# imuncle/TSCM_Calib

Hardware: AMD Instinct MI355X
Metric: LM iterations/sec at 4 cams x 10k views (joint intrinsics+extrinsics, fp64) (higher is better)
Workload: dtype f64

## Files before the change

### tscm_calib_amd/csrc/tscm_kernels.h

```cpp
#pragma once

#include "tscm_math.h"
#include "tscm_fastmath.h"
#include "tscm_nd_plan.h"
#include "tscm_layout.h"
#include "tscm_exec_plan.h"
#include "tscm_columns.h"
#include "tscm_ctrl.h"

namespace tscm {

static_assert(kColFree == kFA && kColGrad == kFR, "tscm_columns.h plans the columns of tscm_math.h's camera tile");
constexpr int kWcolTc = 3;
constexpr int kFac = 56;
constexpr int kFacM = 0;
constexpr int kFacC = 15;
constexpr int kFacL = 21;
constexpr int kFacI = 36;
constexpr int kFacZ = 42;
constexpr int kFacD = 48;
constexpr int kTcols = 15;
constexpr int kTcWb = 0, kTcWc = 4, kTcF = 8, kTcOne = 9, kTcXi = 10, kTcLam = 12, kTcAl = 13, kTcR = 14;
__host__ __device__ constexpr int tc_tc(int j) { return 3 + 4 * j; }
constexpr int kVConst = 27;
// ... 1500 lines not shown
    S.pairpart[(size_t)256 * P.pc_tile[pc] + t] = (red[0][t] + red[1][t]) + (red[2][t] + red[3][t]);
}

template <int ENTRIES>
__device__ __forceinline__ void t_reduce_block(const DevState &S, int bid, int part, int cb, int ce, double (*red)[ENTRIES])
{
    const int e = threadIdx.x % ENTRIES, slice = threadIdx.x / ENTRIES;
    const int entry = part * ENTRIES + e;
    const int per = (ce - cb + kTSlices - 1) / kTSlices;
    const int b0 = cb + slice * per, b1 = min(ce, b0 + per);
    double a0 = 0.0, a1 = 0.0, a2 = 0.0, a3 = 0.0, a4 = 0.0, a5 = 0.0, a6 = 0.0, a7 = 0.0;
    const double *src = S.pairpart + entry;
    for (int c = b0; c < b1; c += 8) {
        const double v0 = src[(size_t)256 * c];
        const double v1 = c + 1 < b1 ? src[(size_t)256 * (c + 1)] : 0.0;
        const double v2 = c + 2 < b1 ? src[(size_t)256 * (c + 2)] : 0.0;
        const double v3 = c + 3 < b1 ? src[(size_t)256 * (c + 3)] : 0.0;
        const double v4 = c + 4 < b1 ? src[(size_t)256 * (c + 4)] : 0.0;
        const double v5 = c + 5 < b1 ? src[(size_t)256 * (c + 5)] : 0.0;
        const double v6 = c + 6 < b1 ? src[(size_t)256 * (c + 6)] : 0.0;
        const double v7 = c + 7 < b1 ? src[(size_t)256 * (c + 7)] : 0.0;
        a0 += v0; a1 += v1; a2 += v2; a3 += v3; a4 += v4; a5 += v5; a6 += v6; a7 += v7;
    }
    red[slice][e] = ((a0 + a1) + (a2 + a3)) + ((a4 + a5) + (a6 + a7));
    __syncthreads();
    if (slice == 0) {
        double v[kTSlices];
#pragma unroll
        for (int q = 0; q < kTSlices; ++q) v[q] = red[q][e];
#pragma unroll
        for (int w = kTSlices / 2; w >= 1; w >>= 1)
#pragma unroll
            for (int q = 0; q < w; ++q) v[q] += v[q + w];
        handoff_store(&S.T[(size_t)256 * bid + entry], v[0]);
    }
}
__global__ __launch_bounds__(kTEntries * kTSlices) void k_T_reduce(DevProblem P, DevState S)
{
    if (S.ctrl->done) return;
    __shared__ double red[kTSlices][kTEntries];
    constexpr int kParts = 256 / kTEntries;
    const int bid = blockIdx.x / kParts;
    t_reduce_block<kTEntries>(S, bid, blockIdx.x % kParts, P.bid_part_ptr[bid], P.bid_part_ptr[bid + 1], red);
}

__device__ __forceinline__ double load_T_lut(const DevProblem &P, const double *T, int i, int j)
{
    int lo = i >> 4, hi = j >> 4, a = i & 15, b = j & 15;
    if (lo > hi) { const int t = lo; lo = hi; hi = t; const int u = a; a = b; b = u; }
    const int tile = P.bid_lut[lo * P.C + hi];
    return tile >= 0 ? T[(size_t)256 * tile + a * 16 + b] : 0.0;
}

struct TailOperands { double x, hg, hrow[kFA]; };
__device__ __forceinline__ void tail_prefetch(const DevProblem &P, const DevState &S, int cur, const double *H, TailOperands &o)
{
    const int i = threadIdx.x;
    o.x = 0.0; o.hg = 0.0;
#pragma unroll
    for (int b = 0; b < kFA; ++b) o.hrow[b] = 0.0;
    if (i < P.n_pad) {
        const int m = i >> 4, ai = i & 15;
        if (ai < 6) o.x = S.cam_rt[cur][6 * m + ai];
        else if (ai < 15) o.x = S.intr[cur][9 * m + (ai - 6)];
        if (ai < kFA) {
#pragma unroll
            for (int b = 0; b < kFA; ++b) o.hrow[b] = H[256 * m + ai * 16 + b];
            o.hg = H[256 * m + ai * 16 + kFR];
        }
    }
}
__device__ __forceinline__ void reduced_solution_tail(const DevProblem &P, const DevState &S, int cur, int fail, const TailOperands &o,
                                                      const double *yv, const double *s_sc, double *s_yh, const unsigned char *s_act, double *sred,
                                                      int publish_epoch = 0)
{
    const int n = P.n_pad, i = threadIdx.x;
    const int m = i >> 4, ai = i & 15;
    double model = 0.0, stepsq = 0.0, yh = 0.0;
    if (i < n) {
        const bool act = s_act[i] && !fail;
        yh = act ? s_sc[i] * yv[i] : 0.0;
        handoff_store(&S.yhat[i], yh);
        s_yh[i] = yh;
        if (ai < kFA) {
            const double x = o.x;
            const double xn = x + (-yh);
            if (ai < 6) handoff_store(&S.cam_rt[cur ^ 1][6 * m + ai], xn); else handoff_store(&S.intr[cur ^ 1][9 * m + (ai - 6)], xn);
            const double d = x - xn; stepsq = d * d;
        } else if (ai < 15) {
            handoff_store(&S.intr[cur ^ 1][9 * m + (ai - 6)], o.x);
        }
    }
    if (publish_epoch > 0) asm volatile("s_waitcnt vmcnt(0)" ::: "memory");
    __syncthreads();
    if (publish_epoch > 0 && i == 0) __hip_atomic_store(S.y_flag, 2 * publish_epoch + (fail ? 1 : 0), __ATOMIC_RELAXED, __HIP_MEMORY_SCOPE_AGENT);
    if (publish_epoch > 0 && i >= 64 && i < 64 + P.C) write_camera_record(S, cur ^ 1, i - 64);
    if (i < n && ai < kFA && yh != 0.0) {
        double hy = 0.0;
#pragma unroll
        for (int b = 0; b < kFA; ++b) hy += o.hrow[b] * s_yh[m * 16 + b];
        model = yh * (o.hg - 0.5 * hy);
    }
    { double red[2] = { model, stepsq }, mdummy = 0.0; block_reduce256<2>(red, mdummy, sred); model = red[0]; stepsq = red[1]; }
    if (i == 0) { S.ctrl->model_cam = model; S.ctrl->stepsq_cam = stepsq; S.ctrl->lin_fail = fail; *S.fac_fail = 0; }
}

template <int NTH, bool WAIT>
__device__ __forceinline__ void backsub_body(const DevProblem &P, const DevState &S, int with_floats, const int blk, const int nblk, const int epoch, const int t_need);

#include "tscm_solve_nd.h"
#include "tscm_solve_dense4.h"

constexpr int kBigNT = 1024;
constexpr int kBigBatch = 4;
__host__ __device__ inline size_t solve_big_lds_bytes(int N, int n_pad)
{
    return sizeof(double) * ((size_t)2 * 16 * (N + 16) + 16 * 17 + 2 * (size_t)N + 16 + 3 * (size_t)n_pad) + sizeof(int) * (size_t)N + (size_t)n_pad;
}
__device__ __forceinline__ size_t big_block(int I, int J) { return ((size_t)(I * (I + 1) / 2 + J)) << 8; }
__device__ __forceinline__ size_t big_idx(int r, int c)
{
    return big_block(r >> 4, c >> 4) + (size_t)((((c & 15) + 16 * (r & 3)) << 2) + ((r & 15) >> 2));
}
__device__ __forceinline__ double readlane_f64(double v, int lane)
{
    return __hiloint2double(__builtin_amdgcn_readlane(__double2hiint(v), lane), __builtin_amdgcn_readlane(__double2loint(v), lane));
}
__device__ __forceinline__ void lds_barrier() { asm volatile("s_waitcnt lgkmcnt(0)\n\ts_barrier" ::: "memory"); }

__global__ __launch_bounds__(kBigNT) void k_solve_reduced_big(DevProblem P, DevState S)
{
    extern __shared__ __attribute__((aligned(32))) double lds[];
    const int n = P.n_pad, na = P.n_act;
    const int N = (na + 15) & ~15, NP = N >> 4;
    const int XP = N + 16;
    double *pbuf = lds;
    double *Ld = pbuf + 2 * 16 * XP;
    double *wv = Ld + 16 * 17;
    double *idg = wv + N;
    double *yk = idg + N;
    double *yv = yk + 16;
    double *s_sc = yv + n;
    double *s_yh = s_sc + n;
    int *s_map = reinterpret_cast<int *>(s_yh + n);
    unsigned char *s_act = reinterpret_cast<unsigned char *>(s_map + N);
    __shared__ int s_fail;
    __shared__ double sred[256];
    const int tid = threadIdx.x, wave = tid >> 6, lane = tid & 63;
    if (S.ctrl->done) return;
    const int cur = S.ctrl->cur;
    const double radius = S.ctrl->radius;
    const double dmin = S.ctrl->opt.min_lm_diagonal, dmax = S.ctrl->opt.max_lm_diagonal;
    const double *H = S.H[cur];
    double *A = S.Abig;
    for (int i = tid; i < n; i += kBigNT) { s_sc[i] = S.s_c[i]; s_act[i] = P.col_active[i]; yv[i] = 0.0; }
    for (int i = tid; i < N; i += kBigNT) s_map[i] = i < na ? P.act_map[i] : -1;
    if (tid == 0) s_fail = S.ctrl->lin_fail | *S.fac_fail;
    __syncthreads();
#ifdef TSCM_BIG_PROFILE
    long long tp0 = wall_clock64(), tp_diag = 0, tp_solve = 0, tp_upd = 0;
#endif
    for (int kb = 0; wave + 16 * kb <= N; kb += 16) {
        const int rmax = min(N, wave + 16 * (kb + 15));
        for (int c = lane; c <= rmax && c < N; c += 64) {
            const int j = s_map[c];
            const int mj = j >> 4, bj = j & 15;
            const double scj = j >= 0 ? s_sc[j] : 0.0;
            double v[16];
#pragma unroll
            for (int u = 0; u < 16; ++u) {
                const int r = wave + 16 * (kb + u);
                v[u] = (r == c) ? 1.0 : 0.0;
                if (r > N || c > r) continue;
                if (r == N) {
                    v[u] = j >= 0 ? scj * (H[256 * mj + bj * 16 + kFR] - load_T_lut(P, S.T, j, mj * 16 + kFR)) : 0.0;
                } else {
                    const int i = s_map[r];
                    if (i >= 0 && j >= 0) {
                        const int mi = i >> 4, ai = i & 15;
// ... 137 lines not shown
        }
        if (wave == 0) {
#pragma unroll
            for (int u = 0; u < 4; ++u) { const int e = lane + 64 * u; Ld[(e >> 4) * 17 + (e & 15)] = ldg[u]; }
            wave_lds_fence();
            if (lane == 0) {
                double y[16];
#pragma unroll
                for (int c = 15; c >= 0; --c) {
                    double v = wv[k0 + c];
#pragma unroll
                    for (int q = c + 1; q < 16; ++q) v -= Ld[q * 17 + c] * y[q];
                    y[c] = v * idg[k0 + c];
                }
#pragma unroll
                for (int c = 0; c < 16; ++c) { yk[c] = y[c]; wv[k0 + c] = y[c]; }
            }
        }
        lds_barrier();
        if (tid < k0) {
            double v = wv[tid];
#pragma unroll
            for (int c = 0; c < 16; ++c) v -= lrow[c] * yk[c];
            wv[tid] = v;
        }
        lds_barrier();
#pragma unroll
        for (int c = 0; c < 16; ++c) lrow[c] = lnext[c];
#pragma unroll
        for (int u = 0; u < 4; ++u) ldg[u] = dnext[u];
    }
    TailOperands tail_ops;
    tail_prefetch(P, S, cur, H, tail_ops);
    for (int i = tid; i < na; i += kBigNT) yv[s_map[i]] = wv[i];
    __syncthreads();
#ifdef TSCM_BIG_PROFILE
    long long tp3 = wall_clock64();
#endif
    reduced_solution_tail(P, S, cur, s_fail, tail_ops, yv, s_sc, s_yh, s_act, sred);
#ifdef TSCM_BIG_PROFILE
    if (tid == 0) printf("big solve N=%d  build %lld  factor %lld (diag %lld solve %lld update %lld)  backsub %lld  tail %lld  [10 ns ticks]\n", N,
                         tp1 - tp0, tp2 - tp1, tp_diag, tp_solve, tp_upd, tp3 - tp2, wall_clock64() - tp3);
#endif
}

constexpr int kBsTile = 64;
template <int NTH> struct BsGeom {
    static constexpr int kBoards = NTH / 8;
    static constexpr int kPassSlots = NTH / 16;
    static constexpr int kPasses = 4;
    static constexpr int kRoundSlots = kPasses * kPassSlots;
    static constexpr int kLdsA = kRoundSlots * 6, kLdsB = kBoards * kFac, kLdsC = kBsTile * (kVFloatOff + 1);
    static constexpr int kLds = kLdsC > kLdsB ? (kLdsC > kLdsA ? kLdsC : kLdsA) : (kLdsB > kLdsA ? kLdsB : kLdsA);
    static_assert(kBoards * kFac == 7 * NTH, "the factor records are 7 doubles per thread");
    static_assert(kBoards <= 64 && 64 + kMaxCam <= NTH, "lane roles of phase B: the boards in wave 0, the cameras from wave 1 on");
};

template <int NTH, bool WAIT>
__device__ __forceinline__ void backsub_body(const DevProblem &P, const DevState &S, int with_floats, const int blk, const int nblk, const int epoch, const int t_need)
{
    constexpr int kBsBoards = BsGeom<NTH>::kBoards, kBsThreads = NTH, kPassSlots = BsGeom<NTH>::kPassSlots, kPasses = BsGeom<NTH>::kPasses, kRoundSlots = BsGeom<NTH>::kRoundSlots;
#ifndef TSCM_BS_CAM_LANE0
#define TSCM_BS_CAM_LANE0 64
#endif
    constexpr int kBsCamLane0 = TSCM_BS_CAM_LANE0;
    const int b0 = blk * kBsBoards;
    const int nbl = min(kBsBoards, P.B - b0);
    const int s0 = P.bv_ptr[b0], s1 = P.bv_ptr[b0 + nbl];
    const int ctrl_done = S.ctrl->done, cur = S.ctrl->cur;
    int fail = WAIT ? 0 : S.ctrl->lin_fail;
    if (ctrl_done) return;
    extern __shared__ __attribute__((aligned(16))) double dyn[];
    double (*s_qv)[6] = reinterpret_cast<double (*)[6]>(dyn);
    double *s_fac = dyn;
    double *st_all = dyn;
    __shared__ double s_q[kBsBoards][6], s_new[kBsBoards][6];
    __shared__ double s_yh[16 * kMaxCam];
    double (*s_rc)[12] = reinterpret_cast<double (*)[12]>(s_yh);
    static_assert(12 * kMaxCam <= 16 * kMaxCam, "s_rc aliases s_yh");
    __shared__ double sm[16];
    __shared__ int s_view[kBsTile];
    const int t = threadIdx.x;
    PHASE_STAMP(ts0);
    const int my_q0 = t < nbl ? P.bv_ptr[b0 + t] : 0, my_q1 = t < nbl ? P.bv_ptr[b0 + t + 1] : 0;
    const int c_slot = min(s0 + t, max(s1 - 1, 0));
    const int c_view = s1 > s0 ? P.slot_view[c_slot] : 0, c_board = s1 > s0 ? P.slot_board[c_slot] : 0, c_cam = s1 > s0 ? P.slot_cam[c_slot] : 0;
    double xb[6], sbv[6];
#pragma unroll
    for (int k = 0; k < 6; ++k) { xb[k] = t < nbl ? S.board_rt[cur][6 * (b0 + t) + k] : 0.0; sbv[k] = t < nbl ? S.s_b[6 * (b0 + t) + k] : 1.0; }
    double facv[7];
#pragma unroll
    for (int j = 0; j < 7; ++j) facv[j] = S.fac[(size_t)kFac * b0 + min(t + kBsThreads * j, nbl * kFac - 1)];
    if constexpr (!WAIT) { for (int i = t; i < P.n_pad; i += kBsThreads) s_yh[i] = S.yhat[i]; }
    if (t < kBsBoards * 6) (&s_q[0][0])[t] = 0.0;
    if constexpr (!WAIT) { if (t == 64) for (int m = blk; m < P.C; m += nblk) write_camera_record(S, cur ^ 1, m); }
    {
        const int grp = t >> 4, a = t & 15;
        const __amdgpu_buffer_rsrc_t r_w = make_rsrc(S.rec[cur], sizeof(double) * (size_t)kRecW * P.V);
        constexpr unsigned BAD = 0xffffe000u;
        double w[kPasses][6];
        int camv[kPasses];
        auto request = [&](int rbase) {
#pragma unroll
            for (int j = 0; j < kPasses; ++j) {
                const int slot = rbase + kPassSlots * j + grp;
                const unsigned off = (a < kFA && slot < s1) ? 8u * ((unsigned)kRecW * (unsigned)slot + 6u * (unsigned)a) : BAD;
#pragma unroll
                for (int k = 0; k < 3; ++k) { const d2 v = buf_load_2f64(r_w, off, 16u * (unsigned)k); w[j][2 * k] = v[0]; w[j][2 * k + 1] = v[1]; }
                camv[j] = P.slot_cam[min(slot, max(s1 - 1, 0))];
            }
        };
        request(s0);
        if constexpr (WAIT) {
            __shared__ int s_flag;
            if (t == 0) {
                const long long t_start = wall_clock64();
                int f;
                while (((f = __hip_atomic_load(S.y_flag, __ATOMIC_RELAXED, __HIP_MEMORY_SCOPE_AGENT)) >> 1) < epoch) {
                    __builtin_amdgcn_s_sleep(8);
                    if (wall_clock64() - t_start > kHandoffTimeoutTicks) { f = -1; break; }
                }
                if (f < 0) {
                    __hip_atomic_store(&S.ctrl->fault, 1, __ATOMIC_RELAXED, __HIP_MEMORY_SCOPE_AGENT);
                    __hip_atomic_store(&S.ctrl->term_type, 2, __ATOMIC_RELAXED, __HIP_MEMORY_SCOPE_AGENT);
                    __hip_atomic_store(&S.ctrl->done, 1, __ATOMIC_RELAXED, __HIP_MEMORY_SCOPE_AGENT);
                }
                s_flag = f;
            }
            __syncthreads();
            if (s_flag < 0 || __hip_atomic_load(&S.ctrl->done, __ATOMIC_RELAXED, __HIP_MEMORY_SCOPE_AGENT)) return;
            fail = s_flag & 1;
            for (int i = t; i < P.n_pad; i += kBsThreads) s_yh[i] = handoff_load(&S.yhat[i]);
        }
        for (int rbase = s0; rbase < s1; rbase += kRoundSlots) {
            const int rend = min(s1, rbase + kRoundSlots);
            __syncthreads();
#pragma unroll
            for (int j = 0; j < kPasses; ++j) {
                const int sl = kPassSlots * j + grp;
                const double yh = a < kFA ? s_yh[16 * camv[j] + a] : 0.0;
                double p[6];
#pragma unroll
                for (int k = 0; k < 6; ++k) {
                    p[k] = (a < kFA ? w[j][k] : 0.0) * yh;
                    p[k] = row16_allsum(p[k]);
                }
                if (a == 0) {
#pragma unroll
                    for (int k = 0; k < 6; ++k) s_qv[sl][k] = p[k];
                }
            }
            if (rbase + kRoundSlots < s1) request(rbase + kRoundSlots);
            __syncthreads();
            if (t < nbl) {
                for (int q = max(my_q0, rbase); q < min(my_q1, rend); ++q)
#pragma unroll
                    for (int k = 0; k < 6; ++k) s_q[t][k] += s_qv[q - rbase][k];
            }
        }
        __syncthreads();
#pragma unroll
        for (int j = 0; j < 7; ++j) s_fac[t + kBsThreads * j] = facv[j];
        __syncthreads();
    }
    PHASE_STAMP(ts1);
    double mb = 0.0, ss = 0.0;
    if (t < nbl) {
        const int b = b0 + t;
        if (my_q1 == my_q0 || fail) {
#pragma unroll
            for (int k = 0; k < 6; ++k) { S.board_rt[cur ^ 1][6 * b + k] = xb[k]; s_new[t][k] = xb[k]; }
        } else {
            const double *f = s_fac + kFac * t;
            double tt[6], y[6], pz[6];
#pragma unroll
            for (int i = 0; i < 6; ++i) {
                double v = f[kFacC + i] * s_q[t][i];
#pragma unroll
                for (int k = 0; k < i; ++k) v -= f[kFacM + i * (i - 1) / 2 + k] * pz[k];
                pz[i] = v;
                tt[i] = f[kFacZ + i] - v;
            }
#pragma unroll
            for (int i = 5; i >= 0; --i) {
                double w = tt[i];
#pragma unroll
                for (int k = i + 1; k < 6; ++k) w -= f[kFacL + k * (k - 1) / 2 + i] * y[k];
                y[i] = w * f[kFacI + i];
            }
#pragma unroll
            for (int k = 0; k < 6; ++k) {
                mb += 0.5 * tt[k] * tt[k] + 0.5 * f[kFacD + k] * y[k] * y[k];
                const double x = xb[k];
                const double xn = x + (-(sbv[k] * y[k]));
                const double d = x - xn;
                ss += d * d;
                S.board_rt[cur ^ 1][6 * b + k] = xn;
                s_new[t][k] = xn;
            }
        }
    } else if (t >= kBsCamLane0 && t < kBsCamLane0 + P.C) {
        const int m = t - kBsCamLane0;
        double crt[3], Rc[9], dRc[27];
        double crt6[6];
#pragma unroll
        for (int k = 0; k < 6; ++k) crt6[k] = WAIT ? handoff_load(&S.cam_rt[cur ^ 1][6 * m + k]) : S.cam_rt[cur ^ 1][6 * m + k];
        for (int k = 0; k < 3; ++k) crt[k] = crt6[k];
        rotation_and_derivatives(crt, Rc, dRc);
        for (int k = 0; k < 9; ++k) s_rc[m][k] = Rc[k];
        for (int k = 0; k < 3; ++k) s_rc[m][9 + k] = crt6[3 + k];

    }
    {
        double red[2] = { mb, ss }, mdummy = 0.0;
        block_reduce256<2>(red, mdummy, sm);
        if (t == 0) { S.bs_part[2 * blk] = red[0]; S.bs_part[2 * blk + 1] = red[1]; }
    }
    PHASE_STAMP(ts2);
    for (int base = s0; base < s1; base += kBsTile) {
        const int slot = base + t;
        int view = -1;
        if (t < kBsTile && slot < s1) {
            const bool first = base == s0;
            view = first ? c_view : P.slot_view[slot];
            const int bl = (first ? c_board : P.slot_board[slot]) - b0, m = first ? c_cam : P.slot_cam[slot];
            double rt[6], bc[kBoardConst];
#pragma unroll
            for (int k = 0; k < 6; ++k) rt[k] = s_new[bl][k];
            board_constants(rt, bc);
            double *o = st_all + (size_t)t * (kVFloatOff + 1);
            view_point_constants(s_rc[m], s_rc[m] + 9, bc, rt + 3, o);
            for (int k = 0; k < 6; ++k) {
                const double d0 = bc[6 + 3 * k], d1 = bc[6 + 3 * k + 1], d2 = bc[6 + 3 * k + 2];
                for (int r = 0; r < 3; ++r) o[9 + 3 * k + r] = s_rc[m][3 * r] * d0 + s_rc[m][3 * r + 1] * d1 + s_rc[m][3 * r + 2] * d2;
            }
            for (int k = kVConst; k < kVFloatOff; ++k) o[k] = 0.0;
        }
        if (t < kBsTile) s_view[t] = view;
        __syncthreads();
        const int nrec = min(kBsTile, s1 - base);
        for (int e = t; e < nrec * kVFloatOff; e += kBsThreads) {
            const int v = e / kVFloatOff, k = e % kVFloatOff;
            S.vconst[(size_t)kVStride * s_view[v] + k] = st_all[(size_t)v * (kVFloatOff + 1) + k];
        }
        if (with_floats) {
            constexpr int kF = kVStride - kVFloatOff;
            for (int e = t; e < nrec * kF; e += kBsThreads) {
                const int v = e / kF, k = e % kF, j = 2 * k;
                const double *sv = st_all + (size_t)v * (kVFloatOff + 1);
                const float f0 = j < kVConst ? (float)sv[j] : 0.f, f1 = j + 1 < kVConst ? (float)sv[j + 1] : 0.f;
                S.vconst[(size_t)kVStride * s_view[v] + kVFloatOff + k] = __hiloint2double(__float_as_int(f1), __float_as_int(f0));
            }
        }
        __syncthreads();
    }
#ifdef TSCM_WAVE_TIMELINE
    if (threadIdx.x == 0 && S.ctrl->iteration == 5 && blk < kKtlGroups) {
        long long *o = g_phs + (size_t)kPhStamps * (kKtlGroups + blk);
        o[0] = ts0; o[1] = ts0; o[2] = ts1; o[3] = ts2; o[4] = wall_clock64(); o[5] = o[4]; o[6] = nbl; o[7] = 0;
// ... 198 lines not shown
```

### tscm_calib_amd/csrc/tscm_solve_dense4.h

```cpp
#pragma once

__device__ __forceinline__ double load_T_small(const DevProblem &P, const double *T, int i, int j)
{
    int lo = i >> 4, hi = j >> 4, a = i & 15, b = j & 15;
    if (lo > hi) { const int t = lo; lo = hi; hi = t; const int u = a; a = b; b = u; }
    const int bit = lo * 8 + hi;
    const unsigned long long m = P.pair_mask;
    const int tile = __popcll(m & ((1ull << bit) - 1ull));
    return ((m >> bit) & 1ull) ? T[256 * tile + a * 16 + b] : 0.0;
}

__host__ __device__ __forceinline__ int kth_set_bit16(unsigned w, int k)
{
    int pos = 0, c;
    c = __builtin_popcount(w & 0xffu); if (k >= c) { k -= c; w >>= 8; pos += 8; }
    c = __builtin_popcount(w & 0xfu);  if (k >= c) { k -= c; w >>= 4; pos += 4; }
    c = __builtin_popcount(w & 0x3u);  if (k >= c) { k -= c; w >>= 2; pos += 2; }
    c = (int)(w & 1u);                 if (k >= c) pos += 1;
    return pos;
}
__device__ __forceinline__ int compact_to_padded(const DevProblem &P, int ci)
{
    int base = 0, q0 = 0;
    unsigned w = P.cam_free[0];
#pragma unroll
    for (int q = 1; q < kMaxCamLds; ++q) { const bool ge = ci >= P.cam_pre[q]; base = ge ? P.cam_pre[q] : base; q0 = ge ? q : q0; w = ge ? P.cam_free[q] : w; }
    return ci < P.n_act ? 16 * q0 + kth_set_bit16(w, ci - base) : -1;
}
template <int TS, int G = 16, int NPD = 64, bool FUSED = false>
__global__ __launch_bounds__((G * G + 63) / 64 * 64, FUSED ? 3 : 1) void k_solve_reduced(DevProblem P, DevState S, int epoch, int withhold, int n_prod, int n_bs, int with_floats)
{
    constexpr int NT = (G * G + 63) / 64 * 64;
    if constexpr (FUSED) {
        static_assert(NT == kFusedEntries * kTSlices, "the T reduction runs in the solver's workgroup shape");
        if ((int)blockIdx.x > n_prod) {
#ifdef TSCM_WAVE_TIMELINE
            KtlScope ktl_bs(5, S.ctrl);
            ktl_bs.blk = (int)blockIdx.x - 1 - n_prod;
#endif
            backsub_body<256, true>(P, S, with_floats, (int)blockIdx.x - 1 - n_prod, n_bs, epoch, epoch * n_prod);
            return;
        }
    }
    KTL(4);
    if constexpr (FUSED) {
        if (blockIdx.x > 0) {
            constexpr int kParts = 256 / kFusedEntries;
            const int bid = ((int)blockIdx.x - 1) / kParts, part = ((int)blockIdx.x - 1) % kParts;
            const int cb = P.bid_part_small[bid], ce = P.bid_part_small[bid + 1];
            if (S.ctrl->done) return;
            __shared__ double red[kTSlices][kFusedEntries];
            t_reduce_block<kFusedEntries>(S, bid, part, cb, ce, red);
            asm volatile("s_waitcnt vmcnt(0)" ::: "memory");
            __syncthreads();
            if (threadIdx.x == 0 && !(withhold && blockIdx.x == 1))
                __hip_atomic_fetch_add(S.t_count, 1, __ATOMIC_RELAXED, __HIP_MEMORY_SCOPE_AGENT);
            return;
        }
    }
    PHASE_STAMP(ts0);
    const int ctrl_done = S.ctrl->done;
    constexpr int N = G * TS;
    constexpr int LD = N + 2;
    extern __shared__ __attribute__((aligned(16))) double lds[];
    double *Lm = lds;
    constexpr int XT = TS * TS + 2;
    double *Xb = Lm + N * LD;
    double *wp = Xb + 2 * G * XT;
    double *idg = wp + N;
    double *yv = idg + N;
    double *s_sc = yv + NPD;
    double *s_yh = s_sc + NPD;
    __shared__ int s_fail;
    __shared__ unsigned char s_act[NPD];
    __shared__ double sred[256];
    const int n = P.n_pad;
    const int tid = threadIdx.x;
    const int NP = (P.n_act + TS - 1) / TS;
    int off[kSolveMapSlots];
#pragma unroll
    for (int q = 0; q < kSolveMapSlots / 4; ++q) {
        const int4 v = P.solve_map[q * NT + tid];
        off[4 * q] = v.x; off[4 * q + 1] = v.y; off[4 * q + 2] = v.z; off[4 * q + 3] = v.w;
    }
    const int ri = off[kMapTile], cj = off[kMapTile + 1];
    const bool mine = off[kMapTile + 2] == 1, rhsrow = off[kMapTile + 2] == 2;
    const int cur = S.ctrl->cur;
    const double radius = S.ctrl->radius;
    const double dmin = S.ctrl->opt.min_lm_diagonal, dmax = S.ctrl->opt.max_lm_diagonal;
    const int ctrl_fail = S.ctrl->lin_fail | *S.fac_fail;
    for (int i = tid; i < NPD; i += NT) { s_sc[i] = i < n ? S.s_c[i] : 1.0; s_act[i] = i < n ? P.col_active[i] : 0; yv[i] = 0.0; }
    if (ctrl_done) return;
    const double *H = S.H[cur];
// ... 152 lines not shown
            load_factor(f, tk);
            load_tile(Ar + ri * XT, ai);
            load_tile(Ar + cj * XT, aj);
            __builtin_amdgcn_sched_barrier(0);
            panel_solve(ai, f, xi);
            if (cj == tk) {
#pragma unroll
                for (int r = 0; r < TS; ++r)
#pragma unroll
                    for (int c = 0; c < TS; ++c) a[r][c] = xi[r][c];
                if (rhsrow) {
#pragma unroll
                    for (int c = 0; c < TS; ++c) wp[tk * TS + c] = xi[0][c];
                }
            } else {
                double xj[TS][TS];
                panel_solve(aj, f, xj);
#pragma unroll
                for (int r = 0; r < TS; ++r)
#pragma unroll
                    for (int c = 0; c < TS; ++c) {
                        double v = a[r][c];
#pragma unroll
                        for (int q = 0; q < TS; ++q) v -= xi[r][q] * xj[c][q];
                        a[r][c] = v;
                    }
            }
        }
        {
            const bool col = cj == tk + 1 && ri > tk + 1 && (mine || rhsrow), dg = ri == tk + 2 && cj == tk + 2 && mine;
            if (col || dg) publish_tile(col ? ArN + ri * XT : s_dt[(tk + 1) & 1], a);
        }
#ifdef TSCM_PHASE_PROFILE
        if (tk == 3 && tid == 11 * G + 5) { asm volatile("" : "+v"(a[3][3])); s_ph[5] = wall_clock64(); }
        if (tk + 1 < NP) __syncthreads();
        if (tk == 3 && tid == 0) { s_ph[6] = wall_clock64(); printf("  panel 3: D x,t %lld  factor %lld | update %lld | to barrier exit %lld\n", s_ph[1] - s_ph[0], s_ph[2] - s_ph[1], s_ph[5] - s_ph[4], s_ph[6] - s_ph[0]); }
#else
        if (tk + 1 < NP) __syncthreads();
#endif
    }
    if (cj < ri && mine) {
#pragma unroll
        for (int r = 0; r < TS; ++r)
#pragma unroll
            for (int c = 0; c < TS; ++c) Lm[(ri * TS + r) * LD + cj * TS + c] = a[r][c];
    }
    __syncthreads();
    PHASE_STAMP(ts2);
#ifdef TSCM_PHASE_PROFILE
    const long long cy2 = clock64();
#endif
    TailOperands tail_ops;
    tail_prefetch(P, S, cur, H, tail_ops);
    if (tid < 64) {
        constexpr int R = (N + 63) / 64;
        double w[R];
#pragma unroll
        for (int q = 0; q < R; ++q) w[q] = tid + 64 * q < NP * TS ? wp[tid + 64 * q] : 0.0;
        for (int tk = NP - 1; tk >= 0; --tk) {
            const int k0 = tk * TS;
            double y[TS];
#pragma unroll
            for (int c = 0; c < TS; ++c) {
                const int k = k0 + c;
                double v = 0.0;
#pragma unroll
                for (int q = 0; q < R; ++q) if ((k >> 6) == q) v = w[q];
                y[c] = __shfl(v, k & 63);
            }
#pragma unroll
            for (int c = TS - 1; c >= 0; --c) {
                double v = y[c];
#pragma unroll
                for (int q = c + 1; q < TS; ++q) v -= Lm[(k0 + q) * LD + k0 + c] * y[q];
                y[c] = v * idg[k0 + c];
            }
#pragma unroll
            for (int q = 0; q < R; ++q) {
                const int i = tid + 64 * q;
                if (i < k0) {
                    double v = w[q];
#pragma unroll
                    for (int c = 0; c < TS; ++c) v -= Lm[(k0 + c) * LD + i] * y[c];
                    w[q] = v;
                } else if (i < k0 + TS) {
#pragma unroll
                    for (int c = 0; c < TS; ++c) if (i == k0 + c) w[q] = y[c];
                }
            }
        }
#pragma unroll
        for (int q = 0; q < R; ++q) { const int pi = tid + 64 * q < N ? compact_to_padded(P, tid + 64 * q) : -1; if (pi >= 0) yv[pi] = w[q]; }
    }
    __syncthreads();
    PHASE_STAMP(ts3);
    reduced_solution_tail(P, S, cur, s_fail, tail_ops, yv, s_sc, s_yh, s_act, sred, FUSED && n_bs > 0 ? epoch : 0);
#ifdef TSCM_PHASE_PROFILE
    if (tid == 0) printf("solve_reduced: ctrl %lld operands %lld  factor %lld (%lld shader clocks)  backsub %lld  tail %lld [10 ns]\n", ts0b - ts0, ts1 - ts0b, ts2 - ts1, cy2 - cy1, ts3 - ts2, wall_clock64() - ts3);
#endif
}
```

### tscm_calib_amd/csrc/tscm_solver.hip

```cpp
#include "tscm/tscm.h"
#include "tscm_host.h"
#include "tscm_kernels.h"
#include "tscm_launch_seq.h"
#include "tscm_mono_batch.h"

#include <hip/hip_runtime.h>
#include <hip/hip_ext.h>
#include <rccl/rccl.h>

#include <algorithm>
#include <chrono>
#include <cstdio>
#include <cstdlib>
#include <cmath>
#include <cstring>
#include <memory>
#include <numeric>
#include <string>
#include <thread>
#include <vector>

using namespace tscm;

static thread_local std::string g_err;
// ... 373 lines not shown
    up(&P.bid_lut, bid_lut); up(&P.board_const, L.board_const);
    s->fixed.assign(C, 0);
    al(&P.col_active, s->n_pad); al(&P.col_ctl, (size_t)16 * kMaxCam); al(&P.act_map, s->n_pad);

    for (int k = 0; k < 2; ++k) {
        al(&S.cam_rt[k], 6 * (size_t)C); al(&S.intr[k], 9 * (size_t)C); al(&S.board_rt[k], 6 * (size_t)B);
        al(&S.rec[k], (size_t)kRec * V); al(&S.H[k], 256 * (size_t)C);
    }
    al(&s->d_init_cam, 6 * (size_t)C); al(&s->d_init_intr, 9 * (size_t)C); al(&s->d_init_board, 6 * (size_t)B);
    al(&s->d_start_cam, 6 * (size_t)C); al(&s->d_start_intr, 9 * (size_t)C); al(&s->d_start_board, 6 * (size_t)B);
    al(&S.board_pc, (size_t)kBoardConst * B); al(&S.cam_pc, (size_t)kCamConst * C); al(&S.vconst, (size_t)kVStride * V);
    al(&S.cconst[0], (size_t)kCStride * C); al(&S.cconst[1], (size_t)kCStride * C);
    al(&S.campart, 512 * (size_t)(P.n_chunks / 4)); al(&S.campart2, 512 * (size_t)C);
    al(&S.H_stage, 256 * (size_t)C + kScal + world);
    al(&S.s_b, 6 * (size_t)B); al(&S.s_c, s->n_pad); al(&S.fac, (size_t)kFac * B);
    al(&S.pairpart, 256 * (size_t)P.n_tiles); al(&S.T, 256 * (size_t)L.n_bids);
    al(&S.t_count, 1); al(&S.y_flag, 1); al(&S.fac_fail, 1);
    al(&S.yhat, s->n_pad);
    S.n_st_blocks = (B + 255) / 256;
    al(&S.bs_part, 2 * (size_t)((B + 15) / 16));
    al(&S.st_part, kStStride * (size_t)S.n_st_blocks);
    S.n_bs_blocks = L.n_bs_blocks;
    al(&S.ctrl, 1); al(&S.ctrl_snap, 1); al(&S.ctl_pub, 1);
    al(&S.stats_count, 64); al(&S.stats_flag, 64);
    HIP_TRY(he);
    for (int *flag : { S.t_count, S.y_flag, S.fac_fail }) HIP_TRY(hipMemset(flag, 0, sizeof(int)));
    HIP_TRY(hipMemset(S.stats_count, 0, 256)); HIP_TRY(hipMemset(S.stats_flag, 0, 256));
    HIP_TRY(hipMemset(S.ctl_pub, 0, sizeof(CtlPub)));
    HIP_TRY(hipMemset(S.T, 0, sizeof(double) * 256 * (size_t)L.n_bids));
    HIP_TRY(hipMemset(S.H_stage, 0, sizeof(double) * (256 * (size_t)C + kScal + world)));
    HIP_TRY(hipMemset(S.campart2, 0, sizeof(double) * 512 * (size_t)C));
    HIP_TRY(hipMemset(S.ctrl, 0, sizeof(Ctrl)));
    HIP_TRY(hipMemset(S.ctrl_snap, 0, sizeof(CtrlHead)));
    HIP_TRY(hipHostMalloc(reinterpret_cast<void **>(&s->h_ctrl), sizeof(Ctrl)));
    HIP_TRY(hipHostGetDevicePointer(reinterpret_cast<void **>(&s->d_h_ctrl), s->h_ctrl, 0));

    s->lds_eval = 4 * lds_eval_bytes;
    s->lds_eval32 = sizeof(double) * (size_t)eval_f32_lds_doubles(p->n_points, g4.ks);
    s->lds_eval4 = lds_eval4; s->eval4 = eval4; s->eval4r = eval4r;
    s->eval32 = f32_kernel(g4.ks, g4.passes > 1, false); s->eval32r = f32_kernel(g4.ks, g4.passes > 1, true);
    if (s->lds_eval32 > 64 * 1024)
        for (EvalKernel k : { s->eval32, s->eval32r }) HIP_TRY(hipFuncSetAttribute(reinterpret_cast<const void *>(k), hipFuncAttributeMaxDynamicSharedMemorySize, (int)s->lds_eval32));
    ColumnPlan cols;
    {
        std::string err;
        if (int rc = plan_columns(L, C, nullptr, cols, err)) return fail(rc, err);
    }
    if (C <= kDense4Cams) {
        int4 *map = nullptr;
        HIP_TRY(s->mem.alloc(&map, (size_t)(kSolveMapSlots / 4) * kSolveMapThreads));
        P.solve_map = map;
        const size_t NN = 64, TT = 4, NPD = 64;
        s->lds_dense4 = sizeof(double) * (NN * (NN + 2) + 2 * (NN / TT) * (TT * TT + 2) + 2 * NN + 3 * NPD);
        int per_cu = 0;
        HIP_TRY(hipOccupancyMaxActiveBlocksPerMultiprocessor(&per_cu, reinterpret_cast<const void *>(k_solve_reduced<4, 16, 64, true>), 256, std::max(s->lds_dense4, s->lds_bs)));
        s->dev.dense4_resident = per_cu * prop.multiProcessorCount;
    }
    if (C > kMaxCamLds) {
        const int NN = (cols.n_act + 15) & ~15;
        const size_t lds_max = solve_big_lds_bytes(NN, s->n_pad);
        HIP_TRY(s->mem.alloc(&S.Abig, (size_t)256 * (NN / 16 + 1) * (NN / 16 + 2) / 2));
        if (lds_max > 64 * 1024) HIP_TRY(hipFuncSetAttribute(reinterpret_cast<const void *>(k_solve_reduced_big), hipFuncAttributeMaxDynamicSharedMemorySize, (int)lds_max));
    }
    if (int rc = apply_columns(s, cols)) return rc;
    if (s->lds_eval > 160 * 1024) return fail(TSCM_E_UNSUPPORTED, "board has too many corners for the LDS board-point tile");
    HIP_TRY(hipDeviceSynchronize());
    *out = sp.release();
    return 0;
}

extern "C" int tscm_solver_create(const tscm_problem *p, int device, tscm_solver **out)
{
    return tscm_solver_create_sharded(p, device, 0, 1, out);
}

static CommKind comm_kind(const tscm_comm *c) { return !c ? kCommNone : c->world > 1 || c->group ? kCommShared : kCommOneRank; }

extern "C" int tscm_solver_debug_withhold_handoff(tscm_solver *s, int on)
{
    if (!s) return fail(TSCM_E_INVALID, "solver is NULL");
    s->withhold_next = on == 3 ? kWithholdStats : on ? kWithholdProducer : 0;
    s->no_rerun_next = on == 2;
    return 0;
}

extern "C" int tscm_solver_reruns(const tscm_solver *s)
{
    if (!s) return fail(TSCM_E_INVALID, "solver is NULL");
    return s->n_reruns;
}

extern "C" int tscm_solver_set_comm(tscm_solver *s, tscm_comm *comm)
{
    if (!s) return fail(TSCM_E_INVALID, "solver is NULL");
    if (comm && comm->device != s->device) return fail(TSCM_E_INVALID, "communicator and solver live on different devices");
    if (comm && (comm->world != s->world || comm->rank != s->rank))
        return fail(TSCM_E_INVALID, "communicator rank / world differ from the solver's shard (tscm_solver_create_sharded)");
    s->comm_reg = comm;
    s->comm = uses_comm(comm_kind(comm), 0) ? comm : nullptr;
    return 0;
}

extern "C" int tscm_solver_upload_params(tscm_solver *s, const double *cam_rt, const double *intr, const double *board_rt)
{
    if (!s || !intr || (!board_rt && s->L.B_total)) return fail(TSCM_E_INVALID, "NULL argument");
    HIP_TRY(hipSetDevice(s->device));
// ... 1212 lines not shown
```

Before: 8718.

## Shorten the dense4 solve-to-backsub handoff critical path

The dense 4-camera reduced solve now does its back-substitution tail step and publishes the y flag from the single wave that did the back-substitution, with no workgroup barrier before the flag. Back-sub operands for the next tile are prefetched into registers, and readlane replaces shuffles. The fused back-substitution blocks get their own LDS region for the factor records, so they can store them while waiting for the flag. They also preload camera extrinsics before the board rounds, which removes barriers after the wait. This shortens the serial latency between solve and backsub, at the cost of more registers and LDS per backsub block and more complex memory-ordering reasoning.

Result: no change. 8683 (-0.4%).

```diff
diff --git a/tscm_calib_amd/csrc/tscm_kernels.h b/tscm_calib_amd/csrc/tscm_kernels.h
--- a/tscm_calib_amd/csrc/tscm_kernels.h
+++ b/tscm_calib_amd/csrc/tscm_kernels.h
@@ -1576,6 +1576,11 @@
     return tile >= 0 ? T[(size_t)256 * tile + a * 16 + b] : 0.0;
 }
 
+__device__ __forceinline__ double readlane_f64(double v, int lane)
+{
+    return __hiloint2double(__builtin_amdgcn_readlane(__double2hiint(v), lane), __builtin_amdgcn_readlane(__double2loint(v), lane));
+}
+
 struct TailOperands { double x, hg, hrow[kFA]; };
 __device__ __forceinline__ void tail_prefetch(const DevProblem &P, const DevState &S, int cur, const double *H, TailOperands &o)
 {
@@ -1594,13 +1599,13 @@
         }
     }
 }
-__device__ __forceinline__ void reduced_solution_tail(const DevProblem &P, const DevState &S, int cur, int fail, const TailOperands &o,
-                                                      const double *yv, const double *s_sc, double *s_yh, const unsigned char *s_act, double *sred,
-                                                      int publish_epoch = 0)
+__device__ __forceinline__ double tail_step(const DevProblem &P, const DevState &S, int cur, int fail, const TailOperands &o,
+                                            const double *yv, const double *s_sc, double *s_yh, const unsigned char *s_act, double &stepsq)
 {
     const int n = P.n_pad, i = threadIdx.x;
     const int m = i >> 4, ai = i & 15;
-    double model = 0.0, stepsq = 0.0, yh = 0.0;
+    double yh = 0.0;
+    stepsq = 0.0;
     if (i < n) {
         const bool act = s_act[i] && !fail;
         yh = act ? s_sc[i] * yv[i] : 0.0;
@@ -1615,9 +1620,14 @@
             handoff_store(&S.intr[cur ^ 1][9 * m + (ai - 6)], o.x);
         }
     }
-    if (publish_epoch > 0) asm volatile("s_waitcnt vmcnt(0)" ::: "memory");
-    __syncthreads();
-    if (publish_epoch > 0 && i == 0) __hip_atomic_store(S.y_flag, 2 * publish_epoch + (fail ? 1 : 0), __ATOMIC_RELAXED, __HIP_MEMORY_SCOPE_AGENT);
+    return yh;
+}
+__device__ __forceinline__ void tail_finish(const DevProblem &P, const DevState &S, int cur, int fail, const TailOperands &o,
+                                            const double *s_yh, double *sred, int publish_epoch, double yh, double stepsq)
+{
+    const int n = P.n_pad, i = threadIdx.x;
+    const int m = i >> 4, ai = i & 15;
+    double model = 0.0;
     if (publish_epoch > 0 && i >= 64 && i < 64 + P.C) write_camera_record(S, cur ^ 1, i - 64);
     if (i < n && ai < kFA && yh != 0.0) {
         double hy = 0.0;
@@ -1628,8 +1638,19 @@
     { double red[2] = { model, stepsq }, mdummy = 0.0; block_reduce256<2>(red, mdummy, sred); model = red[0]; stepsq = red[1]; }
     if (i == 0) { S.ctrl->model_cam = model; S.ctrl->stepsq_cam = stepsq; S.ctrl->lin_fail = fail; *S.fac_fail = 0; }
 }
-
-template <int NTH, bool WAIT>
+__device__ __forceinline__ void reduced_solution_tail(const DevProblem &P, const DevState &S, int cur, int fail, const TailOperands &o,
+                                                      const double *yv, const double *s_sc, double *s_yh, const unsigned char *s_act, double *sred,
+                                                      int publish_epoch = 0)
+{
+    double stepsq;
+    const double yh = tail_step(P, S, cur, fail, o, yv, s_sc, s_yh, s_act, stepsq);
+    if (publish_epoch > 0) asm volatile("s_waitcnt vmcnt(0)" ::: "memory");
+    __syncthreads();
+    if (publish_epoch > 0 && threadIdx.x == 0) __hip_atomic_store(S.y_flag, 2 * publish_epoch + (fail ? 1 : 0), __ATOMIC_RELAXED, __HIP_MEMORY_SCOPE_AGENT);
+    tail_finish(P, S, cur, fail, o, s_yh, sred, publish_epoch, yh, stepsq);
+}
+
+template <int NTH, bool WAIT, bool FAC_OWN = false>
 __device__ __forceinline__ void backsub_body(const DevProblem &P, const DevState &S, int with_floats, const int blk, const int nblk, const int epoch, const int t_need);
 
 #include "tscm_solve_nd.h"
@@ -1645,10 +1666,6 @@
 __device__ __forceinline__ size_t big_idx(int r, int c)
 {
     return big_block(r >> 4, c >> 4) + (size_t)((((c & 15) + 16 * (r & 3)) << 2) + ((r & 15) >> 2));
-}
-__device__ __forceinline__ double readlane_f64(double v, int lane)
-{
-    return __hiloint2double(__builtin_amdgcn_readlane(__double2hiint(v), lane), __builtin_amdgcn_readlane(__double2loint(v), lane));
 }
 __device__ __forceinline__ void lds_barrier() { asm volatile("s_waitcnt lgkmcnt(0)\n\ts_barrier" ::: "memory"); }
 
@@ -1892,11 +1909,12 @@
     static constexpr int kRoundSlots = kPasses * kPassSlots;
     static constexpr int kLdsA = kRoundSlots * 6, kLdsB = kBoards * kFac, kLdsC = kBsTile * (kVFloatOff + 1);
     static constexpr int kLds = kLdsC > kLdsB ? (kLdsC > kLdsA ? kLdsC : kLdsA) : (kLdsB > kLdsA ? kLdsB : kLdsA);
+    static constexpr int kLdsFacOwn = kLds + kLdsB;
     static_assert(kBoards * kFac == 7 * NTH, "the factor records are 7 doubles per thread");
     static_assert(kBoards <= 64 && 64 + kMaxCam <= NTH, "lane roles of phase B: the boards in wave 0, the cameras from wave 1 on");
 };
 
-template <int NTH, bool WAIT>
+template <int NTH, bool WAIT, bool FAC_OWN>
 __device__ __forceinline__ void backsub_body(const DevProblem &P, const DevState &S, int with_floats, const int blk, const int nblk, const int epoch, const int t_need)
 {
     constexpr int kBsBoards = BsGeom<NTH>::kBoards, kBsThreads = NTH, kPassSlots = BsGeom<NTH>::kPassSlots, kPasses = BsGeom<NTH>::kPasses, kRoundSlots = BsGeom<NTH>::kRoundSlots;
@@ -1912,7 +1930,8 @@
     if (ctrl_done) return;
     extern __shared__ __attribute__((aligned(16))) double dyn[];
     double (*s_qv)[6] = reinterpret_cast<double (*)[6]>(dyn);
-    double *s_fac = dyn;
+    constexpr bool kFacOwn = WAIT && FAC_OWN;
+    double *s_fac = kFacOwn ? dyn + BsGeom<NTH>::kLds : dyn;
     double *st_all = dyn;
     __shared__ double s_q[kBsBoards][6], s_new[kBsBoards][6];
     __shared__ double s_yh[16 * kMaxCam];
@@ -1934,6 +1953,8 @@
     if constexpr (!WAIT) { for (int i = t; i < P.n_pad; i += kBsThreads) s_yh[i] = S.yhat[i]; }
     if (t < kBsBoards * 6) (&s_q[0][0])[t] = 0.0;
     if constexpr (!WAIT) { if (t == 64) for (int m = blk; m < P.C; m += nblk) write_camera_record(S, cur ^ 1, m); }
+    double crt6[6] = { 0.0, 0.0, 0.0, 0.0, 0.0, 0.0 };
+    const bool cam_lane = t >= kBsCamLane0 && t < kBsCamLane0 + P.C;
     {
         const int grp = t >> 4, a = t & 15;
         const __amdgpu_buffer_rsrc_t r_w = make_rsrc(S.rec[cur], sizeof(double) * (size_t)kRecW * P.V);
@@ -1953,6 +1974,10 @@
         request(s0);
         if constexpr (WAIT) {
             __shared__ int s_flag;
+            if constexpr (kFacOwn) {
+#pragma unroll
+                for (int j = 0; j < 7; ++j) s_fac[t + kBsThreads * j] = facv[j];
+            }
             if (t == 0) {
                 const long long t_start = wall_clock64();
                 int f;
@@ -1970,6 +1995,10 @@
             __syncthreads();
             if (s_flag < 0 || __hip_atomic_load(&S.ctrl->done, __ATOMIC_RELAXED, __HIP_MEMORY_SCOPE_AGENT)) return;
             fail = s_flag & 1;
+            if (cam_lane) {
+#pragma unroll
+                for (int k = 0; k < 6; ++k) crt6[k] = handoff_load(&S.cam_rt[cur ^ 1][6 * (t - kBsCamLane0) + k]);
+            }
             for (int i = t; i < P.n_pad; i += kBsThreads) s_yh[i] = handoff_load(&S.yhat[i]);
         }
         for (int rbase = s0; rbase < s1; rbase += kRoundSlots) {
@@ -1998,10 +2027,14 @@
                     for (int k = 0; k < 6; ++k) s_q[t][k] += s_qv[q - rbase][k];
             }
         }
-        __syncthreads();
-#pragma unroll
-        for (int j = 0; j < 7; ++j) s_fac[t + kBsThreads * j] = facv[j];
-        __syncthreads();
+        if constexpr (kFacOwn) {
+            if (s1 == s0) __syncthreads();
+        } else {
+            __syncthreads();
+#pragma unroll
+            for (int j = 0; j < 7; ++j) s_fac[t + kBsThreads * j] = facv[j];
+            __syncthreads();
+        }
     }
     PHASE_STAMP(ts1);
     double mb = 0.0, ss = 0.0;
@@ -2039,12 +2072,13 @@
                 s_new[t][k] = xn;
             }
         }
-    } else if (t >= kBsCamLane0 && t < kBsCamLane0 + P.C) {
+    } else if (cam_lane) {
         const int m = t - kBsCamLane0;
         double crt[3], Rc[9], dRc[27];
-        double crt6[6];
-#pragma unroll
-        for (int k = 0; k < 6; ++k) crt6[k] = WAIT ? handoff_load(&S.cam_rt[cur ^ 1][6 * m + k]) : S.cam_rt[cur ^ 1][6 * m + k];
+        if constexpr (!WAIT) {
+#pragma unroll
+            for (int k = 0; k < 6; ++k) crt6[k] = S.cam_rt[cur ^ 1][6 * m + k];
+        }
         for (int k = 0; k < 3; ++k) crt[k] = crt6[k];
         rotation_and_derivatives(crt, Rc, dRc);
         for (int k = 0; k < 9; ++k) s_rc[m][k] = Rc[k];
diff --git a/tscm_calib_amd/csrc/tscm_solve_dense4.h b/tscm_calib_amd/csrc/tscm_solve_dense4.h
--- a/tscm_calib_amd/csrc/tscm_solve_dense4.h
+++ b/tscm_calib_amd/csrc/tscm_solve_dense4.h
@@ -38,7 +38,7 @@
             KtlScope ktl_bs(5, S.ctrl);
             ktl_bs.blk = (int)blockIdx.x - 1 - n_prod;
 #endif
-            backsub_body<256, true>(P, S, with_floats, (int)blockIdx.x - 1 - n_prod, n_bs, epoch, epoch * n_prod);
+            backsub_body<256, true, true>(P, S, with_floats, (int)blockIdx.x - 1 - n_prod, n_bs, epoch, epoch * n_prod);
             return;
         }
     }
@@ -297,13 +297,33 @@
 #endif
     TailOperands tail_ops;
     tail_prefetch(P, S, cur, H, tail_ops);
+    constexpr bool kWavePublish = NPD == 64;
+    const int publish_epoch = FUSED && n_bs > 0 ? epoch : 0;
+    double t_yh = 0.0, t_stepsq = 0.0;
     if (tid < 64) {
         constexpr int R = (N + 63) / 64;
         double w[R];
 #pragma unroll
         for (int q = 0; q < R; ++q) w[q] = tid + 64 * q < NP * TS ? wp[tid + 64 * q] : 0.0;
+        struct StepOps { double dg[TS][TS], id[TS], lc[R][TS]; };
+        auto load_step = [&](StepOps &o, int tk) {
+            const int k0 = tk * TS;
+#pragma unroll
+            for (int c = 0; c < TS; ++c) {
+                o.id[c] = idg[k0 + c];
+#pragma unroll
+                for (int q = c + 1; q < TS; ++q) o.dg[q][c] = Lm[(k0 + q) * LD + k0 + c];
+#pragma unroll
+                for (int q = 0; q < R; ++q) o.lc[q][c] = tid + 64 * q < k0 ? Lm[(k0 + c) * LD + tid + 64 * q] : 0.0;
+            }
+        };
+        StepOps nxt;
+        load_step(nxt, max(NP - 1, 0));
         for (int tk = NP - 1; tk >= 0; --tk) {
             const int k0 = tk * TS;
+            const StepOps op = nxt;
+            load_step(nxt, max(tk - 1, 0));
+            __builtin_amdgcn_sched_barrier(0);
             double y[TS];
 #pragma unroll
             for (int c = 0; c < TS; ++c) {
@@ -311,14 +331,14 @@
                 double v = 0.0;
 #pragma unroll
                 for (int q = 0; q < R; ++q) if ((k >> 6) == q) v = w[q];
-                y[c] = __shfl(v, k & 63);
+                y[c] = readlane_f64(v, k & 63);
             }
 #pragma unroll
             for (int c = TS - 1; c >= 0; --c) {
                 double v = y[c];
 #pragma unroll
-                for (int q = c + 1; q < TS; ++q) v -= Lm[(k0 + q) * LD + k0 + c] * y[q];
-                y[c] = v * idg[k0 + c];
+                for (int q = c + 1; q < TS; ++q) v -= op.dg[q][c] * y[q];
+                y[c] = v * op.id[c];
             }
 #pragma unroll
             for (int q = 0; q < R; ++q) {
@@ -326,7 +346,7 @@
                 if (i < k0) {
                     double v = w[q];
 #pragma unroll
-                    for (int c = 0; c < TS; ++c) v -= Lm[(k0 + c) * LD + i] * y[c];
+                    for (int c = 0; c < TS; ++c) v -= op.lc[q][c] * y[c];
                     w[q] = v;
                 } else if (i < k0 + TS) {
 #pragma unroll
@@ -336,10 +356,25 @@
         }
 #pragma unroll
         for (int q = 0; q < R; ++q) { const int pi = tid + 64 * q < N ? compact_to_padded(P, tid + 64 * q) : -1; if (pi >= 0) yv[pi] = w[q]; }
+        if constexpr (kWavePublish) {
+            __builtin_amdgcn_fence(__ATOMIC_RELEASE, "wavefront");
+            __builtin_amdgcn_wave_barrier();
+            __builtin_amdgcn_fence(__ATOMIC_ACQUIRE, "wavefront");
+            PHASE_STAMP(ts3w);
+            t_yh = tail_step(P, S, cur, s_fail, tail_ops, yv, s_sc, s_yh, s_act, t_stepsq);
+            if (publish_epoch > 0) {
+                asm volatile("s_waitcnt vmcnt(0)" ::: "memory");
+                if (tid == 0) __hip_atomic_store(S.y_flag, 2 * publish_epoch + (s_fail ? 1 : 0), __ATOMIC_RELAXED, __HIP_MEMORY_SCOPE_AGENT);
+            }
+#ifdef TSCM_PHASE_PROFILE
+            if (tid == 0) printf("solve_reduced: backsub (one wave) %lld  step to flag %lld [10 ns]\n", ts3w - ts2, wall_clock64() - ts3w);
+#endif
+        }
     }
     __syncthreads();
     PHASE_STAMP(ts3);
-    reduced_solution_tail(P, S, cur, s_fail, tail_ops, yv, s_sc, s_yh, s_act, sred, FUSED && n_bs > 0 ? epoch : 0);
+    if constexpr (kWavePublish) tail_finish(P, S, cur, s_fail, tail_ops, s_yh, sred, publish_epoch, t_yh, t_stepsq);
+    else reduced_solution_tail(P, S, cur, s_fail, tail_ops, yv, s_sc, s_yh, s_act, sred, publish_epoch);
 #ifdef TSCM_PHASE_PROFILE
     if (tid == 0) printf("solve_reduced: ctrl %lld operands %lld  factor %lld (%lld shader clocks)  backsub %lld  tail %lld [10 ns]\n", ts0b - ts0, ts1 - ts0b, ts2 - ts1, cy2 - cy1, ts3 - ts2, wall_clock64() - ts3);
 #endif
diff --git a/tscm_calib_amd/csrc/tscm_solver.hip b/tscm_calib_amd/csrc/tscm_solver.hip
--- a/tscm_calib_amd/csrc/tscm_solver.hip
+++ b/tscm_calib_amd/csrc/tscm_solver.hip
@@ -449,6 +449,7 @@
         P.solve_map = map;
         const size_t NN = 64, TT = 4, NPD = 64;
         s->lds_dense4 = sizeof(double) * (NN * (NN + 2) + 2 * (NN / TT) * (TT * TT + 2) + 2 * NN + 3 * NPD);
+        static_assert(BsGeom<256>::kLdsFacOwn <= NN * (NN + 2) + 2 * (NN / TT) * (TT * TT + 2) + 2 * NN + 3 * NPD, "the riders' dynamic LDS fits the solver workgroup's");
         int per_cu = 0;
         HIP_TRY(hipOccupancyMaxActiveBlocksPerMultiprocessor(&per_cu, reinterpret_cast<const void *>(k_solve_reduced<4, 16, 64, true>), 256, std::max(s->lds_dense4, s->lds_bs)));
         s->dev.dense4_resident = per_cu * prop.multiProcessorCount;
```
